# MoFHeka/MeepoEmbedding

Hardware: AMD Instinct MI355X
Metric: key-lookups/sec (higher is better)
Workload: dtype int64 keys / fp32 rows (copy)

## Files before the change

include/meepo_embedding.h:

```cpp
#ifndef MEEPO_EMBEDDING_H
#define MEEPO_EMBEDDING_H
#include <stddef.h>
#include <stdint.h>

#ifdef __cplusplus
extern "C" {
#endif

#define MEE_ABI_VERSION 2

#define MEE_EMPTY_KEY     INT64_MIN
#define MEE_RECLAIMED_KEY (INT64_MIN + 1)
#define MEE_BUCKET_WIDTH  16

enum { MEE_OK = 0, MEE_ERR_INVALID_ARG = -1, MEE_ERR_OUT_OF_MEMORY = -2, MEE_ERR_HIP = -3,
       MEE_ERR_NO_DEVICE = -4, MEE_ERR_BATCH_TOO_LARGE = -5, MEE_ERR_UNSUPPORTED = -6,
       MEE_ERR_RCCL = -7  };

enum { MEE_OPT_NONE = 0, MEE_OPT_ADAGRAD = 1, MEE_OPT_ADAM = 2 };
enum { MEE_INIT_CONSTANT = 0, MEE_INIT_UNIFORM = 1 };
enum { MEE_STATUS_TABLE_FULL = 1u, MEE_STATUS_RESERVED_KEY = 2u, MEE_STATUS_STALE_HANDLE = 4u, MEE_STATUS_INTERNAL = 8u };
enum { MEE_MEM_HBM = 0, MEE_MEM_HOST_PINNED = 1 };
enum { MEE_FLAG_TRACK_HITS = 1u, MEE_FLAG_ADMISSION = 2u };

// ... 153 lines not shown
int mee_apply_adam_indexed(mee_table* t, const int64_t* d_keys, const float* d_grads, size_t n_grad_rows, const uint32_t* d_grad_index,
                           size_t n, float lr, float beta1, float beta2, float eps, uint64_t step, void* stream);
int mee_apply_prepare(mee_table* t, const int64_t* d_keys, size_t n, void* stream);
int mee_apply_discard(mee_table* t, void* stream);
int mee_dedup_sum(mee_table* t, const int64_t* d_keys, const float* d_grads, size_t n, int64_t* d_uniq_out,
                  float* d_gsum_out, uint32_t* d_counts_out, int64_t* d_inverse_out, int64_t miss_index,
                  void* stream);

int mee_dedup_keys(mee_table* t, const int64_t* d_keys, size_t n, int64_t* d_uniq_out, int64_t* d_inverse_out, int64_t miss_index,
                   void* stream);

int mee_hash_batch(const int64_t* d_keys, size_t n, uint64_t n_buckets, uint32_t n_shards, uint64_t* d_mix_out,
                   uint64_t* d_bucket_out, uint32_t* d_owner_out, void* stream);
int mee_router_create(int32_t device, uint64_t max_batch, uint32_t n_shards, mee_router** out);
int mee_router_destroy(mee_router* r);
int mee_partition(mee_router* r, const int64_t* d_keys, size_t n, int64_t* d_send_keys, uint64_t* d_counts,
                  int64_t* d_perm, void* stream);
int mee_partition_padded(mee_router* r, const int64_t* d_keys, size_t n, int64_t* d_send_keys, uint64_t* d_counts,
                         int64_t* d_perm, void* stream);
int mee_scatter_rows(const void* d_rows, const int64_t* d_perm, size_t n, size_t row_bytes, void* d_out,
                     void* stream);
int mee_gather_rows(const void* d_rows, const int64_t* d_perm, size_t n, size_t row_bytes, void* d_out,
                    void* stream);

int mee_p2p_create(int32_t device, uint32_t n_shards, uint32_t rank, uint64_t slots_per_peer, uint64_t max_batch, uint32_t dim,
                   int with_payload, mee_p2p** out);
int mee_p2p_destroy(mee_p2p* c);
#define MEE_P2P_BUFFERS 6
int mee_p2p_export(mee_p2p* c, void* handles );
int mee_p2p_connect(mee_p2p* c, const void* all_handles );
int mee_p2p_buffers(mee_p2p* c, float** d_out, uint8_t** d_found);
int mee_p2p_push(mee_p2p* c, mee_router* r, const int64_t* d_send_keys, const int64_t* d_perm, const uint64_t* d_counts, size_t n,
                 void* stream);
int mee_p2p_find(mee_p2p* c, const mee_table* t, void* stream);
int mee_p2p_push_rows(mee_p2p* c, mee_router* r, const int64_t* d_send_keys, const int64_t* d_perm, const uint64_t* d_counts,
                      const float* d_rows, size_t n, void* stream);
int mee_p2p_inbox(mee_p2p* c, int64_t** d_keys, float** d_rows, uint64_t* n_slots);
int mee_p2p_barrier(mee_p2p* c, void* stream);
int mee_p2p_status(mee_p2p* c, uint32_t* bits_out, void* stream);


#define MEE_COMM_ID_BYTES 128
int mee_comm_unique_id(void* id_out );
int mee_comm_create(const void* id, uint32_t n_ranks, uint32_t rank, int32_t device, void** comm_out);
int mee_comm_destroy(void* comm);
int mee_comm_aborted(void* comm);
int mee_sharded_create(mee_table* local, void* nccl_comm, uint64_t max_batch ,
                       double pad_slack, mee_sharded** out);
enum { MEE_SHARDED_DEDUP = 1u };
typedef struct mee_sharded_options {
    uint32_t struct_size;
    uint32_t flags;
    uint64_t max_batch;
    double   pad_slack;
    mee_table* cold;
    uint64_t hot_key_limit;
} mee_sharded_options;
int mee_sharded_create_ex(mee_table* local, void* nccl_comm, const mee_sharded_options* options, mee_sharded** out);
int mee_sharded_destroy(mee_sharded* s);
int mee_sharded_info(const mee_sharded* s, uint32_t* n_shards, uint32_t* rank, uint64_t* segment_capacity );
int mee_sharded_find(mee_sharded* s, const int64_t* d_keys, size_t n, float* d_out, uint8_t* d_found , void* stream);
int mee_sharded_find_or_insert(mee_sharded* s, const int64_t* d_keys, size_t n, float* d_out, uint8_t* d_found, void* stream);
int mee_sharded_find_as(mee_sharded* s, const int64_t* d_keys, size_t n, void* d_out, uint32_t out_dtype, uint8_t* d_found , void* stream);
int mee_sharded_find_or_insert_as(mee_sharded* s, const int64_t* d_keys, size_t n, void* d_out, uint32_t out_dtype, uint8_t* d_found, void* stream);
int mee_sharded_traffic(const mee_sharded* s, uint64_t* sent_bytes, uint64_t* received_bytes);
int mee_sharded_insert(mee_sharded* s, const int64_t* d_keys, const float* d_values, size_t n, void* stream);
int mee_sharded_assign(mee_sharded* s, const int64_t* d_keys, const float* d_values, size_t n, uint8_t* d_found, void* stream);
int mee_sharded_remove(mee_sharded* s, const int64_t* d_keys, size_t n, uint8_t* d_found, void* stream);
int mee_sharded_apply_adagrad(mee_sharded* s, const int64_t* d_keys, const float* d_grads, size_t n, float lr, float eps, void* stream);
int mee_sharded_apply_adam(mee_sharded* s, const int64_t* d_keys, const float* d_grads, size_t n, float lr, float beta1, float beta2,
// ... 10 lines not shown
```

include/meepo_embedding.hpp:

```cpp
#pragma once
#include <cstdint>
#include <stdexcept>
#include <string>
#include <utility>

#include "meepo_embedding.h"

namespace meepo {

class Error : public std::runtime_error {
public:
    Error(int code, const std::string& msg) : std::runtime_error("meepo error " + std::to_string(code) + ": " + msg), code_(code) {}
    int code() const noexcept { return code_; }
private:
    int code_;
};

inline void check(int rc) {
    if (rc != MEE_OK) throw Error(rc, mee_last_error());
}

struct TableOptions {
    int32_t device = 0;
    uint64_t capacity = 0;
// ... 142 lines not shown
    }
    size_t size(void* stream = nullptr) const { return hot_.size(stream) + cold_.size(stream); }
private:
    Table hot_, cold_;
};

class Router {
public:
    Router(int32_t device, uint64_t max_batch, uint32_t n_shards) { check(mee_router_create(device, max_batch, n_shards, &r_)); }
    ~Router() { if (r_) mee_router_destroy(r_); }
    Router(Router&& o) noexcept : r_(std::exchange(o.r_, nullptr)) {}
    Router(const Router&) = delete;
    Router& operator=(const Router&) = delete;
    mee_router* handle() const noexcept { return r_; }
    void partition(const int64_t* d_keys, size_t n, int64_t* d_send_keys, uint64_t* d_counts, int64_t* d_perm, void* stream = nullptr) { check(mee_partition(r_, d_keys, n, d_send_keys, d_counts, d_perm, stream)); }
    void partition_padded(const int64_t* d_keys, size_t n, int64_t* d_send_keys, uint64_t* d_counts, int64_t* d_perm, void* stream = nullptr) { check(mee_partition_padded(r_, d_keys, n, d_send_keys, d_counts, d_perm, stream)); }
    static void scatter_rows(const void* d_rows, const int64_t* d_perm, size_t n, size_t row_bytes, void* d_out, void* stream = nullptr) { check(mee_scatter_rows(d_rows, d_perm, n, row_bytes, d_out, stream)); }
    static void gather_rows(const void* d_rows, const int64_t* d_perm, size_t n, size_t row_bytes, void* d_out, void* stream = nullptr) { check(mee_gather_rows(d_rows, d_perm, n, row_bytes, d_out, stream)); }
private:
    mee_router* r_ = nullptr;
};

class PeerExchange {
public:
    PeerExchange(int32_t device, uint32_t n_shards, uint32_t rank, uint64_t slots_per_peer, uint64_t max_batch, uint32_t dim, bool with_payload = false) {
        check(mee_p2p_create(device, n_shards, rank, slots_per_peer, max_batch, dim, with_payload ? 1 : 0, &c_));
    }
    ~PeerExchange() { if (c_) mee_p2p_destroy(c_); }
    PeerExchange(const PeerExchange&) = delete;
    PeerExchange& operator=(const PeerExchange&) = delete;
    void export_handles(void* handles_6x64) { check(mee_p2p_export(c_, handles_6x64)); }
    void connect(const void* all_handles_rank_major) { check(mee_p2p_connect(c_, all_handles_rank_major)); }
    void push(Router& r, const int64_t* d_send_keys, const int64_t* d_perm, const uint64_t* d_counts, size_t n, void* stream = nullptr) { check(mee_p2p_push(c_, r.handle(), d_send_keys, d_perm, d_counts, n, stream)); }
    void find(const Table& t, void* stream = nullptr) { check(mee_p2p_find(c_, t.handle(), stream)); }
    void barrier(void* stream = nullptr) { check(mee_p2p_barrier(c_, stream)); }
    void push_rows(Router& r, const int64_t* d_send_keys, const int64_t* d_perm, const uint64_t* d_counts, const float* d_rows, size_t n, void* stream = nullptr) {
        check(mee_p2p_push_rows(c_, r.handle(), d_send_keys, d_perm, d_counts, d_rows, n, stream));
    }
    int64_t* inbox_keys() const { int64_t* k = nullptr; check(mee_p2p_inbox(c_, &k, nullptr, nullptr)); return k; }
    float* inbox_rows() const { float* r = nullptr; check(mee_p2p_inbox(c_, nullptr, &r, nullptr)); return r; }
    uint64_t inbox_slots() const { uint64_t n = 0; check(mee_p2p_inbox(c_, nullptr, nullptr, &n)); return n; }
    float* rows() const { float* o = nullptr; check(mee_p2p_buffers(c_, &o, nullptr)); return o; }
    uint8_t* found() const { uint8_t* f = nullptr; check(mee_p2p_buffers(c_, nullptr, &f)); return f; }
    uint32_t status(void* stream = nullptr) { uint32_t b = 0; check(mee_p2p_status(c_, &b, stream)); return b; }
private:
    mee_p2p* c_ = nullptr;
};

class Communicator {
public:
    static void unique_id(void* id_128_bytes) { check(mee_comm_unique_id(id_128_bytes)); }
    Communicator(const void* id_128_bytes, uint32_t n_ranks, uint32_t rank, int32_t device) { check(mee_comm_create(id_128_bytes, n_ranks, rank, device, &c_)); }
    ~Communicator() { if (c_) mee_comm_destroy(c_); }
    Communicator(const Communicator&) = delete;
    Communicator& operator=(const Communicator&) = delete;
    void* handle() const noexcept { return c_; }
private:
    void* c_ = nullptr;
};

class ShardedTable {
public:
    ShardedTable(Table& local, void* nccl_comm, uint64_t max_batch, double pad_slack = 0.0) { check(mee_sharded_create(local.handle(), nccl_comm, max_batch, pad_slack, &s_)); }
    ShardedTable(Table& local, void* nccl_comm, uint64_t max_batch, double pad_slack, Table* cold, uint32_t flags = 0, uint64_t hot_key_limit = 0) {
        mee_sharded_options o{};
        o.struct_size = sizeof o; o.flags = flags; o.max_batch = max_batch; o.pad_slack = pad_slack; o.cold = cold ? cold->handle() : nullptr; o.hot_key_limit = hot_key_limit;
        check(mee_sharded_create_ex(local.handle(), nccl_comm, &o, &s_));
    }
    ~ShardedTable() { if (s_) mee_sharded_destroy(s_); }
    ShardedTable(const ShardedTable&) = delete;
    ShardedTable& operator=(const ShardedTable&) = delete;
    void find(const int64_t* d_keys, size_t n, float* d_out, uint8_t* d_found = nullptr, void* stream = nullptr) { check(mee_sharded_find(s_, d_keys, n, d_out, d_found, stream)); }
    void find_or_insert(const int64_t* d_keys, size_t n, float* d_out, uint8_t* d_found = nullptr, void* stream = nullptr) { check(mee_sharded_find_or_insert(s_, d_keys, n, d_out, d_found, stream)); }
// ... 17 lines not shown
```

meepoembedding_amd/_lib.py:

```python
from __future__ import annotations

import ctypes as C
import os

import torch

_HERE = os.path.dirname(os.path.abspath(__file__))
LIB_PATH = os.environ.get("MEE_LIB_PATH") or os.path.join(_HERE, "libmeepo_hip.so")

OK = 0
ERR_INVALID_ARG, ERR_OUT_OF_MEMORY, ERR_HIP, ERR_NO_DEVICE, ERR_BATCH_TOO_LARGE, ERR_UNSUPPORTED, ERR_RCCL = -1, -2, -3, -4, -5, -6, -7
OPT_NONE, OPT_ADAGRAD, OPT_ADAM = 0, 1, 2
INIT_CONSTANT, INIT_UNIFORM = 0, 1
STATUS_TABLE_FULL, STATUS_RESERVED_KEY, STATUS_STALE_HANDLE, STATUS_INTERNAL = 1, 2, 4, 8
FIND_DEFAULT, FIND_STREAM_STORES, FIND_CACHED_STORES, FIND_STREAM_ROWS, FIND_STREAM_BUCKETS = 0, 1, 2, 4, 8
HANDLE_SLOT_MASK = (1 << 40) - 1
MEM_HBM, MEM_HOST_PINNED = 0, 1
DTYPE_F32, DTYPE_BF16 = 0, 1
FLAG_TRACK_HITS, FLAG_ADMISSION = 1, 2
ABI_VERSION = 2
EMPTY_KEY = -(1 << 63)
RECLAIMED_KEY = EMPTY_KEY + 1
BUCKET_WIDTH = 16

# ... 99 lines not shown
    "mee_find_located": (C.c_int, [_vp, _vp, _sz, _vp, _vp, _vp, _vp]),
    "mee_find_or_insert_located": (C.c_int, [_vp, _vp, _sz, _vp, _vp, _vp, _vp]),
    "mee_find_located_prepare": (C.c_int, [_vp, _vp, _sz, _vp, _vp, _vp, _vp]),
    "mee_find_or_insert_located_prepare": (C.c_int, [_vp, _vp, _sz, _vp, _vp, _vp, _vp]),
    "mee_apply_adagrad_located": (C.c_int, [_vp, _vp, _vp, _vp, _sz, _f32, _f32, _vp]),
    "mee_apply_adam_located": (C.c_int, [_vp, _vp, _vp, _vp, _sz, _f32, _f32, _f32, _f32, _u64, _vp]),
    "mee_find_or_insert_admit": (C.c_int, [_vp, _vp, _sz, _vp, _vp, _u32, _vp]),
    "mee_admission_decay": (C.c_int, [_vp, _u32, _vp]),
    "mee_locate": (C.c_int, [_vp, _vp, _sz, _vp, _vp, _vp]),
    "mee_table_plane": (C.c_int, [_vp, _u32, C.POINTER(_vp), C.POINTER(_u64), C.POINTER(_u32)]),
    "mee_device_calibration": (C.c_int, [C.c_int32, C.POINTER(Calibration)]),
    "mee_probe_length": (C.c_int, [_vp, _vp, _sz, C.POINTER(_u64), _vp]),
    "mee_probe_histogram": (C.c_int, [_vp, _vp, _sz, C.POINTER(C.c_uint64), _vp]),
    "mee_apply_adagrad": (C.c_int, [_vp, _vp, _vp, _sz, _f32, _f32, _vp]),
    "mee_apply_adam": (C.c_int, [_vp, _vp, _vp, _sz, _f32, _f32, _f32, _f32, _u64, _vp]),
    "mee_apply_prepare": (C.c_int, [_vp, _vp, _sz, _vp]),
    "mee_apply_discard": (C.c_int, [_vp, _vp]),
    "mee_dedup_sum": (C.c_int, [_vp, _vp, _vp, _sz, _vp, _vp, _vp, _vp, C.c_int64, _vp]),
    "mee_hash_batch": (C.c_int, [_vp, _sz, _u64, _u32, _vp, _vp, _vp, _vp]),
    "mee_router_create": (C.c_int, [_i32, _u64, _u32, C.POINTER(_vp)]),
    "mee_router_destroy": (C.c_int, [_vp]),
    "mee_partition_padded": (C.c_int, [_vp, _vp, _sz, _vp, _vp, _vp, _vp]),
    "mee_partition": (C.c_int, [_vp, _vp, _sz, _vp, _vp, _vp, _vp]),
    "mee_p2p_create": (C.c_int, [_i32, _u32, _u32, _u64, _u64, _u32, C.c_int, C.POINTER(_vp)]),
    "mee_p2p_barrier": (C.c_int, [_vp, _vp]),
    "mee_p2p_push_rows": (C.c_int, [_vp, _vp, _vp, _vp, _vp, _vp, _sz, _vp]),
    "mee_p2p_inbox": (C.c_int, [_vp, C.POINTER(_vp), C.POINTER(_vp), C.POINTER(_u64)]),
    "mee_p2p_destroy": (C.c_int, [_vp]),
    "mee_p2p_export": (C.c_int, [_vp, _vp]),
    "mee_p2p_connect": (C.c_int, [_vp, _vp]),
    "mee_p2p_buffers": (C.c_int, [_vp, C.POINTER(_vp), C.POINTER(_vp)]),
    "mee_p2p_push": (C.c_int, [_vp, _vp, _vp, _vp, _vp, _sz, _vp]),
    "mee_p2p_find": (C.c_int, [_vp, _vp, _vp]),
    "mee_p2p_status": (C.c_int, [_vp, C.POINTER(_u32), _vp]),
    "mee_scatter_rows": (C.c_int, [_vp, _vp, _sz, _sz, _vp, _vp]),
    "mee_gather_rows": (C.c_int, [_vp, _vp, _sz, _sz, _vp, _vp]),
    "mee_comm_unique_id": (C.c_int, [_vp]),
    "mee_comm_create": (C.c_int, [_vp, _u32, _u32, _i32, C.POINTER(_vp)]),
    "mee_comm_destroy": (C.c_int, [_vp]),
    "mee_comm_aborted": (C.c_int, [_vp]),
    "mee_sharded_create": (C.c_int, [_vp, _vp, _u64, C.c_double, C.POINTER(_vp)]),
    "mee_sharded_create_ex": (C.c_int, [_vp, _vp, C.POINTER(ShardedOptions), C.POINTER(_vp)]),
    "mee_sharded_clear_status": (C.c_int, [_vp, _vp]),
    "mee_sharded_destroy": (C.c_int, [_vp]),
    "mee_sharded_info": (C.c_int, [_vp, C.POINTER(_u32), C.POINTER(_u32), C.POINTER(_u64)]),
    "mee_sharded_find": (C.c_int, [_vp, _vp, _sz, _vp, _vp, _vp]),
    "mee_sharded_find_or_insert": (C.c_int, [_vp, _vp, _sz, _vp, _vp, _vp]),
    "mee_sharded_find_as": (C.c_int, [_vp, _vp, _sz, _vp, _u32, _vp, _vp]),
    "mee_sharded_find_or_insert_as": (C.c_int, [_vp, _vp, _sz, _vp, _u32, _vp, _vp]),
    "mee_sharded_traffic": (C.c_int, [_vp, C.POINTER(_u64), C.POINTER(_u64)]),
    "mee_sharded_insert": (C.c_int, [_vp, _vp, _vp, _sz, _vp]),
    "mee_sharded_assign": (C.c_int, [_vp, _vp, _vp, _sz, _vp, _vp]),
    "mee_sharded_remove": (C.c_int, [_vp, _vp, _sz, _vp, _vp]),
    "mee_sharded_apply_adagrad": (C.c_int, [_vp, _vp, _vp, _sz, _f32, _f32, _vp]),
    "mee_sharded_apply_adam": (C.c_int, [_vp, _vp, _vp, _sz, _f32, _f32, _f32, _f32, _u64, _vp]),
    "mee_sharded_size": (C.c_int, [_vp, C.POINTER(_sz), _vp]),
    "mee_sharded_status": (C.c_int, [_vp, C.POINTER(_u32), _vp]),
}

_lib = None


def lib() -> C.CDLL:
    global _lib
    if _lib is None:
        if not os.path.exists(LIB_PATH):
# ... 29 lines not shown
```

meepoembedding_amd/csrc/meepo_router.hip:

```cpp
#include <hip/hip_runtime.h>

#include <cstdlib>
#include <cstring>
#include <new>

#include "meepo_device.h"
#include "meepo_host.h"

struct mee_router {
    int device;
    uint64_t max_batch;
    uint32_t n_shards;
    uint32_t max_blocks;
    uint32_t* blockcnt;
    uint64_t* base;
};

struct mee_p2p {
    int device;
    uint32_t n_shards, rank, dim;
    uint64_t cap, max_batch;
    int64_t* inbox_keys;
    int32_t* inbox_dst;
    uint32_t* inbox_cnt;
    float* out;
    uint8_t* found;
    float* inbox_rows;
    uint32_t* status;
    void** d_tables;
    void* h_tables[6][64];
    bool connected;
};

namespace mee {

constexpr int kPartBlock = 1024;
constexpr int kMaxShards = 64;

__global__ void hash_batch_kernel(const int64_t* __restrict__ keys, uint64_t n, uint64_t nb, uint32_t g, uint64_t* mix_out,
                                  uint64_t* bucket_out, uint32_t* owner_out) {
    for (uint64_t i = blockIdx.x * (uint64_t)blockDim.x + threadIdx.x; i < n; i += (uint64_t)gridDim.x * blockDim.x) {
        const int64_t k = keys[i];
        if (mix_out) mix_out[i] = mix64((uint64_t)k);
        if (bucket_out) bucket_out[i] = bucket_of(k, nb);
        if (owner_out) owner_out[i] = owner_of(k, g);
    }
}

template <bool SKIP_PAD>
__global__ __launch_bounds__(kPartBlock) void part_count_kernel(const int64_t* __restrict__ keys, uint32_t n, uint32_t g,
                                                                uint32_t* blockcnt) {
    __shared__ uint32_t wcnt[kPartBlock / 64][kMaxShards];
    const uint32_t i = blockIdx.x * kPartBlock + threadIdx.x;
    const int lane = threadIdx.x & 63, w = threadIdx.x >> 6;
    const int64_t key = i < n ? keys[i] : kEmpty;
    const bool inb = i < n && !(SKIP_PAD && key == kEmpty);
    const uint32_t o = inb ? owner_of(key, g) : 0xFFFFFFFFu;
    for (uint32_t p = 0; p < g; ++p) {
        const uint64_t m = __ballot(o == p);
        if (lane == 0) wcnt[w][p] = (uint32_t)__popcll(m);
    }
    __syncthreads();
    if (threadIdx.x < g) {
        uint32_t c = 0;
#pragma unroll
        for (int ww = 0; ww < kPartBlock / 64; ++ww) c += wcnt[ww][threadIdx.x];
        blockcnt[(uint64_t)blockIdx.x * g + threadIdx.x] = c;
    }
}

__global__ __launch_bounds__(1024) void part_scan_kernel(uint32_t* blockcnt, uint32_t n_blocks, uint32_t g, uint64_t* base,
                                                         uint64_t* counts_out) {
    __shared__ uint64_t total[kMaxShards];
    const int lane = threadIdx.x & 63, w = threadIdx.x >> 6, nw = blockDim.x >> 6;
    for (uint32_t p = w; p < g; p += nw) {
        uint32_t run = 0;
        for (uint32_t b0 = 0; b0 < n_blocks; b0 += 64) {
            const uint32_t b = b0 + lane;
            const uint32_t c = b < n_blocks ? blockcnt[(uint64_t)b * g + p] : 0;
            uint32_t incl = c;
#pragma unroll
            for (int d = 1; d < 64; d <<= 1) {
                const uint32_t t = __shfl_up(incl, d);
                if (lane >= d) incl += t;
            }
            if (b < n_blocks) blockcnt[(uint64_t)b * g + p] = run + incl - c;
            run += __shfl(incl, 63);
        }
        if (lane == 0) total[p] = run;
    }
    __syncthreads();
    if (threadIdx.x == 0) {
        uint64_t acc = 0;
        for (uint32_t p = 0; p < g; ++p) {
            base[p] = acc;
            counts_out[p] = total[p];
            acc += total[p];
        }
    }
}

template <bool SKIP_PAD>
__global__ __launch_bounds__(kPartBlock) void part_scatter_kernel(const int64_t* __restrict__ keys, uint32_t n, uint32_t g,
                                                                  const uint32_t* __restrict__ blockoff,
                                                                  const uint64_t* __restrict__ base, int64_t* send_keys,
                                                                  int64_t* perm) {
    __shared__ uint32_t wcnt[kPartBlock / 64][kMaxShards];
    const uint32_t i = blockIdx.x * kPartBlock + threadIdx.x;
    const int lane = threadIdx.x & 63, w = threadIdx.x >> 6;
    const int64_t key = i < n ? keys[i] : kEmpty;
    const bool inb = i < n && !(SKIP_PAD && key == kEmpty);
    const uint32_t o = inb ? owner_of(key, g) : 0xFFFFFFFFu;
    uint32_t r = 0;
    for (uint32_t p = 0; p < g; ++p) {
        const uint64_t m = __ballot(o == p);
        if (o == p) r = (uint32_t)__popcll(m & ((1ull << lane) - 1));
        if (lane == 0) wcnt[w][p] = (uint32_t)__popcll(m);
    }
    __syncthreads();
    if (inb) {
        for (int ww = 0; ww < w; ++ww) r += wcnt[ww][o];
        const uint64_t dst = base[o] + blockoff[(uint64_t)blockIdx.x * g + o] + r;
        send_keys[dst] = key;
        perm[dst] = (int64_t)i;
    }
}

template <typename T, bool SCATTER>
__global__ void permute_rows_kernel(const T* __restrict__ rows, const int64_t* __restrict__ perm, uint64_t n, uint32_t epr,
                                    T* __restrict__ out) {
    const uint64_t total = n * epr;
    for (uint64_t idx = blockIdx.x * (uint64_t)blockDim.x + threadIdx.x; idx < total; idx += (uint64_t)gridDim.x * blockDim.x) {
        const uint64_t q = idx / epr;
        const uint32_t e = (uint32_t)(idx - q * epr);
        const uint64_t p = (uint64_t)perm[q];
        if (SCATTER) out[p * epr + e] = rows[idx];
        else out[idx] = rows[p * epr + e];
    }
}

template <bool SCATTER>
static int permute_rows(const void* d_rows, const int64_t* d_perm, size_t n, size_t row_bytes, void* d_out, void* stream,
                        const char* name) {
    if (n && (!d_rows || !d_perm || !d_out)) return fail(MEE_ERR_INVALID_ARG, "%s: null argument", name);
    if (n == 0 || row_bytes == 0) return MEE_OK;
    hipStream_t st = (hipStream_t)stream;
    const bool a16 = row_bytes % 16 == 0 && ((uintptr_t)d_rows % 16 == 0) && ((uintptr_t)d_out % 16 == 0);
    const bool a4 = row_bytes % 4 == 0 && ((uintptr_t)d_rows % 4 == 0) && ((uintptr_t)d_out % 4 == 0);
    if (a16) {
        const uint32_t epr = (uint32_t)(row_bytes / 16);
        permute_rows_kernel<float4, SCATTER><<<grid_for(n * epr, 256, 1u << 16), 256, 0, st>>>((const float4*)d_rows, d_perm, n, epr, (float4*)d_out);
    } else if (a4) {
        const uint32_t epr = (uint32_t)(row_bytes / 4);
        permute_rows_kernel<uint32_t, SCATTER><<<grid_for(n * epr, 256, 1u << 16), 256, 0, st>>>((const uint32_t*)d_rows, d_perm, n, epr, (uint32_t*)d_out);
    } else {
        const uint32_t epr = (uint32_t)row_bytes;
        permute_rows_kernel<uint8_t, SCATTER><<<grid_for(n * epr, 256, 1u << 16), 256, 0, st>>>((const uint8_t*)d_rows, d_perm, n, epr, (uint8_t*)d_out);
    }
    MEE_HIP(hipGetLastError());
    return MEE_OK;
}

constexpr int kP2PBuffers = 6;
struct P2PPeers {
    int64_t** keys; int32_t** dst; uint32_t** cnt; float** out; uint8_t** found; float** rows;
};

__global__ __launch_bounds__(256) void p2p_push_kernel(const int64_t* __restrict__ send_keys, const int64_t* __restrict__ perm,
                                                       const uint64_t* __restrict__ counts, const uint64_t* __restrict__ base,
                                                       P2PPeers peers, uint32_t me, uint64_t cap, uint32_t* status, int pad) {
    const uint32_t p = blockIdx.y;
    const uint64_t cnt = counts[p];
    const uint64_t take = cnt < cap ? cnt : cap;
    int64_t* __restrict__ dk = peers.keys[p] + (uint64_t)me * cap;
    int32_t* __restrict__ dd = peers.dst[p] + (uint64_t)me * cap;
    const uint64_t b0 = base[p];
    for (uint64_t j = blockIdx.x * (uint64_t)blockDim.x + threadIdx.x; j < take; j += (uint64_t)gridDim.x * blockDim.x) {
        dk[j] = send_keys[b0 + j];
        dd[j] = (int32_t)perm[b0 + j];
    }
    if (pad)
        for (uint64_t j = take + blockIdx.x * (uint64_t)blockDim.x + threadIdx.x; j < cap; j += (uint64_t)gridDim.x * blockDim.x) dk[j] = kEmpty;
    if (blockIdx.x == 0 && threadIdx.x == 0) {
        peers.cnt[p][me] = (uint32_t)take;
        if (cnt > cap) atomicOr(status, 1u);
    }
}

__global__ __launch_bounds__(64) void p2p_barrier_kernel(P2PPeers peers, uint32_t me, uint32_t n_shards, uint32_t* status,
                                                         unsigned long long timeout_ticks) {
    const uint32_t q = threadIdx.x;
    uint32_t epoch = 0;
    if (q == 0) { epoch = status[1] + 1; status[1] = epoch; }
    epoch = __shfl(epoch, 0);
    if (q < n_shards) {
        uint32_t* theirs = peers.cnt[q] + n_shards + me;
        __hip_atomic_store(theirs, epoch, __ATOMIC_RELEASE, __HIP_MEMORY_SCOPE_SYSTEM);
        const uint32_t* mine = peers.cnt[me] + n_shards + q;
        const unsigned long long t0 = wall_clock64();
        while ((int32_t)(__hip_atomic_load(mine, __ATOMIC_ACQUIRE, __HIP_MEMORY_SCOPE_SYSTEM) - epoch) < 0) {
            if (wall_clock64() - t0 > timeout_ticks) { atomicOr(status, 2u); break; }
            __builtin_amdgcn_s_sleep(8);
        }
    }
}

__global__ __launch_bounds__(256) void p2p_push_rows_kernel(const float4* __restrict__ rows, const int64_t* __restrict__ perm,
                                                            const uint64_t* __restrict__ counts, const uint64_t* __restrict__ base,
                                                            P2PPeers peers, uint32_t me, uint64_t cap, uint32_t dim4) {
    const int lane = threadIdx.x & 63, tile = lane >> 4, tl = lane & 15;
    const uint32_t p = blockIdx.y;
    const uint64_t cnt = counts[p];
    const uint64_t take = cnt < cap ? cnt : cap;
    float4* __restrict__ dr = reinterpret_cast<float4*>(peers.rows[p]) + (uint64_t)me * cap * dim4;
    const uint64_t b0 = base[p];
    const uint64_t wave = (uint64_t)blockIdx.x * (blockDim.x >> 6) + (threadIdx.x >> 6), n_waves = (uint64_t)gridDim.x * (blockDim.x >> 6);
    for (uint64_t j0 = wave * 4; j0 < take; j0 += n_waves * 4) {
        const uint64_t j = j0 + tile;
// ... 136 lines not shown
static int partition_common(mee_router* r, const int64_t* d_keys, size_t n, int64_t* d_send_keys, uint64_t* d_counts, int64_t* d_perm,
                            void* stream, bool skip_pad, const char* name) {
    if (!r || !d_counts || (n && (!d_keys || !d_send_keys || !d_perm))) return fail(MEE_ERR_INVALID_ARG, "%s: null argument", name);
    if (n > r->max_batch) return fail(MEE_ERR_BATCH_TOO_LARGE, "%s: n=%zu exceeds max_batch=%llu", name, n, (unsigned long long)r->max_batch);
    DeviceGuard g(r->device);
    hipStream_t st = (hipStream_t)stream;
    const uint32_t nblk = (uint32_t)((n + kPartBlock - 1) / kPartBlock);
    if (nblk) with_flag(skip_pad, [&](auto sp) { part_count_kernel<sp><<<nblk, kPartBlock, 0, st>>>(d_keys, (uint32_t)n, r->n_shards, r->blockcnt); });
    part_scan_kernel<<<1, 1024, 0, st>>>(r->blockcnt, nblk, r->n_shards, r->base, d_counts);
    if (nblk) with_flag(skip_pad, [&](auto sp) { part_scatter_kernel<sp><<<nblk, kPartBlock, 0, st>>>(d_keys, (uint32_t)n, r->n_shards, r->blockcnt, r->base, d_send_keys, d_perm); });
    MEE_HIP(hipGetLastError());
    return MEE_OK;
}
int mee_partition(mee_router* r, const int64_t* d_keys, size_t n, int64_t* d_send_keys, uint64_t* d_counts, int64_t* d_perm,
                  void* stream) {
    MEE_RANGE("mee_partition");
    return partition_common(r, d_keys, n, d_send_keys, d_counts, d_perm, stream, false, "mee_partition");
}
int mee_partition_padded(mee_router* r, const int64_t* d_keys, size_t n, int64_t* d_send_keys, uint64_t* d_counts, int64_t* d_perm,
                         void* stream) {
    MEE_RANGE("mee_partition_padded");
    return partition_common(r, d_keys, n, d_send_keys, d_counts, d_perm, stream, true, "mee_partition_padded");
}

int mee_p2p_destroy(mee_p2p* c) {
    MEE_RANGE("mee_p2p_destroy");
    if (!c) return MEE_OK;
    DeviceGuard g(c->device);
    (void)hipDeviceSynchronize();
    if (c->connected)
        for (int b = 0; b < kP2PBuffers; ++b)
            for (uint32_t p = 0; p < c->n_shards; ++p)
                if (p != c->rank && c->h_tables[b][p]) (void)hipIpcCloseMemHandle(c->h_tables[b][p]);
    void* mine[] = {c->inbox_keys, c->inbox_dst, c->inbox_cnt, c->out, c->found, c->inbox_rows, c->status, c->d_tables};
    for (void* p : mine) if (p) (void)hipFree(p);
    delete c;
    return MEE_OK;
}

int mee_p2p_create(int32_t device, uint32_t n_shards, uint32_t rank, uint64_t slots_per_peer, uint64_t max_batch, uint32_t dim,
                   int with_payload, mee_p2p** out) {
    MEE_RANGE("mee_p2p_create");
    if (!out) return fail(MEE_ERR_INVALID_ARG, "mee_p2p_create: null out");
    *out = nullptr;
    if (n_shards == 0 || n_shards > (uint32_t)kMaxShards || rank >= n_shards || slots_per_peer == 0 || max_batch == 0 ||
        max_batch > (1ull << 30) || dim < 4 || (dim & 3))
        return fail(MEE_ERR_INVALID_ARG, "mee_p2p_create: bad arguments");
    int ndev = 0;
    if (hipGetDeviceCount(&ndev) != hipSuccess || ndev <= 0) return fail(MEE_ERR_NO_DEVICE, "mee_p2p_create: no HIP device visible");
    if (device < 0 || device >= ndev) return fail(MEE_ERR_INVALID_ARG, "mee_p2p_create: device %d out of range", device);
    DeviceGuard g(device);
    mee_p2p* c = new (std::nothrow) mee_p2p();
    if (!c) return fail(MEE_ERR_OUT_OF_MEMORY, "host allocation failed");
    memset(c, 0, sizeof *c);
    c->device = device; c->n_shards = n_shards; c->rank = rank; c->dim = dim; c->cap = slots_per_peer; c->max_batch = max_batch;
    const uint64_t slots = (uint64_t)n_shards * slots_per_peer;
    const bool fine = getenv("MEE_P2P_COARSE") == nullptr;
    auto sym_alloc = [&](void** p, size_t bytes) {
        return fine ? hipExtMallocWithFlags(p, bytes, hipDeviceMallocFinegrained) : hipMalloc(p, bytes);
    };
    if (sym_alloc((void**)&c->inbox_keys, slots * 8) != hipSuccess || sym_alloc((void**)&c->inbox_dst, slots * 4) != hipSuccess ||
        sym_alloc((void**)&c->inbox_cnt, 2 * n_shards * 4) != hipSuccess || sym_alloc((void**)&c->out, (max_batch + 1) * (uint64_t)dim * 4) != hipSuccess ||
        sym_alloc((void**)&c->found, max_batch + 1) != hipSuccess ||
        (with_payload && sym_alloc((void**)&c->inbox_rows, slots * (uint64_t)dim * 4) != hipSuccess) ||
        hipMalloc((void**)&c->status, 8) != hipSuccess ||
        hipMalloc((void**)&c->d_tables, kP2PBuffers * (size_t)n_shards * sizeof(void*)) != hipSuccess) {
        mee_p2p_destroy(c);
        return fail(MEE_ERR_OUT_OF_MEMORY, "mee_p2p_create: device allocation failed (%s)", fine ? "fine-grained" : "coarse-grained");
    }
    if (hipMemset(c->inbox_cnt, 0, 2 * n_shards * 4) != hipSuccess || hipMemset(c->status, 0, 8) != hipSuccess) {
        mee_p2p_destroy(c);
        return fail(MEE_ERR_HIP, "mee_p2p_create: hipMemset failed");
    }
    *out = c;
    return MEE_OK;
}

static void* p2p_local(const mee_p2p* c, int b) {
    switch (b) { case 0: return c->inbox_keys; case 1: return c->inbox_dst; case 2: return c->inbox_cnt; case 3: return c->out; case 4: return c->found; default: return c->inbox_rows; }
}

int mee_p2p_export(mee_p2p* c, void* handles) {
    MEE_RANGE("mee_p2p_export");
    if (!c || !handles) return fail(MEE_ERR_INVALID_ARG, "mee_p2p_export: null argument");
    static_assert(sizeof(hipIpcMemHandle_t) == MEE_IPC_HANDLE_BYTES, "IPC handle size");
    DeviceGuard g(c->device);
    memset(handles, 0, (size_t)kP2PBuffers * MEE_IPC_HANDLE_BYTES);
    for (int b = 0; b < kP2PBuffers; ++b) {
        if (!p2p_local(c, b)) continue;
        hipIpcMemHandle_t h;
        MEE_HIP(hipIpcGetMemHandle(&h, p2p_local(c, b)));
        memcpy((char*)handles + b * MEE_IPC_HANDLE_BYTES, &h, MEE_IPC_HANDLE_BYTES);
    }
    return MEE_OK;
}

int mee_p2p_connect(mee_p2p* c, const void* all_handles) {
    MEE_RANGE("mee_p2p_connect");
    if (!c || !all_handles) return fail(MEE_ERR_INVALID_ARG, "mee_p2p_connect: null argument");
    if (c->connected) return fail(MEE_ERR_INVALID_ARG, "mee_p2p_connect: already connected");
    DeviceGuard g(c->device);
    for (uint32_t p = 0; p < c->n_shards; ++p)
        for (int b = 0; b < kP2PBuffers; ++b) {
// ... 11 lines not shown
}

int mee_p2p_buffers(mee_p2p* c, float** d_out, uint8_t** d_found) {
    if (!c) return fail(MEE_ERR_INVALID_ARG, "mee_p2p_buffers: null argument");
    if (d_out) *d_out = c->out;
    if (d_found) *d_found = c->found;
    return MEE_OK;
}

static P2PPeers p2p_peers(const mee_p2p* c) {
    P2PPeers pp;
    pp.keys = (int64_t**)(c->d_tables + 0 * (size_t)c->n_shards);
    pp.dst = (int32_t**)(c->d_tables + 1 * (size_t)c->n_shards);
    pp.cnt = (uint32_t**)(c->d_tables + 2 * (size_t)c->n_shards);
    pp.out = (float**)(c->d_tables + 3 * (size_t)c->n_shards);
    pp.found = (uint8_t**)(c->d_tables + 4 * (size_t)c->n_shards);
    pp.rows = (float**)(c->d_tables + 5 * (size_t)c->n_shards);
    return pp;
}

int mee_p2p_push(mee_p2p* c, mee_router* r, const int64_t* d_send_keys, const int64_t* d_perm, const uint64_t* d_counts, size_t n,
                 void* stream) {
    MEE_RANGE("mee_p2p_push");
    if (!c || !r || !d_counts || (n && (!d_send_keys || !d_perm))) return fail(MEE_ERR_INVALID_ARG, "mee_p2p_push: null argument");
    if (!c->connected) return fail(MEE_ERR_INVALID_ARG, "mee_p2p_push: not connected");
    if (r->n_shards != c->n_shards || n > c->max_batch) return fail(MEE_ERR_INVALID_ARG, "mee_p2p_push: router/batch mismatch");
    DeviceGuard g(c->device);
    const dim3 grid(grid_for(n / c->n_shards + 256, 256, 1024), c->n_shards);
    p2p_push_kernel<<<grid, 256, 0, (hipStream_t)stream>>>(d_send_keys, d_perm, d_counts, r->base, p2p_peers(c), c->rank, c->cap, c->status, 0);
    MEE_HIP(hipGetLastError());
    return MEE_OK;
}

int mee_p2p_push_rows(mee_p2p* c, mee_router* r, const int64_t* d_send_keys, const int64_t* d_perm, const uint64_t* d_counts,
                      const float* d_rows, size_t n, void* stream) {
    MEE_RANGE("mee_p2p_push_rows");
    if (!c || !r || !d_counts || (n && (!d_send_keys || !d_perm))) return fail(MEE_ERR_INVALID_ARG, "mee_p2p_push_rows: null argument");
    if (!c->connected || !c->inbox_rows) return fail(MEE_ERR_INVALID_ARG, "mee_p2p_push_rows: context not connected or created without payload");
    if (r->n_shards != c->n_shards || n > c->max_batch) return fail(MEE_ERR_INVALID_ARG, "mee_p2p_push_rows: router/batch mismatch");
    DeviceGuard g(c->device);
    hipStream_t st = (hipStream_t)stream;
    const dim3 gk(grid_for(c->cap, 256, 1024), c->n_shards);
    p2p_push_kernel<<<gk, 256, 0, st>>>(d_send_keys, d_perm, d_counts, r->base, p2p_peers(c), c->rank, c->cap, c->status, 1);
    if (d_rows) {
        const dim3 gr(grid_for(n / c->n_shards + 64, 16, 4096), c->n_shards);
        p2p_push_rows_kernel<<<gr, 256, 0, st>>>((const float4*)d_rows, d_perm, d_counts, r->base, p2p_peers(c), c->rank, c->cap, c->dim / 4);
    }
    MEE_HIP(hipGetLastError());
    return MEE_OK;
}

int mee_p2p_inbox(mee_p2p* c, int64_t** d_keys, float** d_rows, uint64_t* n_slots) {
    if (!c) return fail(MEE_ERR_INVALID_ARG, "mee_p2p_inbox: null argument");
    if (d_keys) *d_keys = c->inbox_keys;
    if (d_rows) *d_rows = c->inbox_rows;
    if (n_slots) *n_slots = (uint64_t)c->n_shards * c->cap;
    return MEE_OK;
}

int mee_p2p_find(mee_p2p* c, const mee_table* t, void* stream) {
    MEE_RANGE("mee_p2p_find");
    if (!c || !t) return fail(MEE_ERR_INVALID_ARG, "mee_p2p_find: null argument");
    if (!c->connected) return fail(MEE_ERR_INVALID_ARG, "mee_p2p_find: not connected");
    const TableView v = table_view(t);
    if (v.dim != c->dim || v.device != c->device) return fail(MEE_ERR_INVALID_ARG, "mee_p2p_find: table dim/device mismatch");
    DeviceGuard g(c->device);
    const dim3 grid(grid_for(c->cap, 32, 1u << 16), c->n_shards);
    hipStream_t st = (hipStream_t)stream;
    with_row_shape(v.dim4, [&](auto d4) {
        p2p_find_kernel<d4, RowShape<d4>::rows_per_tile><<<grid, 256, 0, st>>>(v.keys, (const float4*)v.values, v.nb, v.dim4, v.default_value, c->inbox_keys,
                                                                               c->inbox_dst, c->inbox_cnt, p2p_peers(c), c->cap);
    });
    MEE_HIP(hipGetLastError());
    return MEE_OK;
}

int mee_p2p_barrier(mee_p2p* c, void* stream) {
    MEE_RANGE("mee_p2p_barrier");
    if (!c) return fail(MEE_ERR_INVALID_ARG, "mee_p2p_barrier: null argument");
    if (!c->connected) return fail(MEE_ERR_INVALID_ARG, "mee_p2p_barrier: not connected");
    DeviceGuard g(c->device);
    p2p_barrier_kernel<<<1, 64, 0, (hipStream_t)stream>>>(p2p_peers(c), c->rank, c->n_shards, c->status, 500000000ull);
    MEE_HIP(hipGetLastError());
    return MEE_OK;
}

int mee_p2p_status(mee_p2p* c, uint32_t* bits_out, void* stream) {
    MEE_RANGE("mee_p2p_status");
    if (!c || !bits_out) return fail(MEE_ERR_INVALID_ARG, "mee_p2p_status: null argument");
// ... 17 lines not shown
```

meepoembedding_amd/p2p.py:

```python
from __future__ import annotations

import ctypes as C

import torch
import torch.distributed as dist

from . import _lib
from ._lib import check


class _Raw:

    def __init__(self, ptr: int, shape, typestr: str):
        self.__cuda_array_interface__ = {"shape": tuple(shape), "typestr": typestr, "data": (ptr, False), "version": 2}


class PeerShardedFind:
    def __init__(self, local, router, max_batch: int, group=None, slack: float = 1.25, payload: bool = False,
                 device_barrier: bool = True):
        self.local, self.router, self.group = local, router, group
        self.world, self.rank = dist.get_world_size(group), dist.get_rank(group)
        self.device, self.dim, self.max_batch = local.device, local.dim, max_batch
        if router.n_shards != self.world:
            raise ValueError("router shards != process group size")
# ... 43 lines not shown
        if int(ok.item()) == 0:
            if self._h:
                _lib.lib().mee_p2p_destroy(self._h)
                self._h = None
            raise _lib.MeepoError(_lib.ERR_HIP, f"peer-to-peer set-up failed on some rank during {what}: {err!r}")

    def close(self) -> None:
        if getattr(self, "_h", None):
            try:
                self._barrier()
            except Exception:
                pass
            _lib.lib().mee_p2p_destroy(self._h)
            self._h = None

    def _barrier(self) -> None:
        if self.device_barrier and self._h:
            check(_lib.lib().mee_p2p_barrier(self._h, torch.cuda.current_stream(self.device).cuda_stream))
        elif self._staged:
            torch.cuda.synchronize(self.device)
            dist.barrier(group=self.group)
        else:
            dist.all_reduce(self._tok, group=self.group)

    def find(self, keys: torch.Tensor, check_overflow: bool = True, dedup: bool = False):
        keys = keys.contiguous().view(-1)
        n = keys.numel()
        if n > self.max_batch:
            raise _lib.MeepoError(_lib.ERR_BATCH_TOO_LARGE, f"n={n} exceeds max_batch={self.max_batch}")
        L = _lib.lib()
        s = torch.cuda.current_stream(self.device).cuda_stream
        if dedup:
            uniq, inverse = self.local.dedup_keys(keys, miss_index=self.max_batch)
            send_keys, counts, perm = self.router.partition(uniq, skip_padding=True)
            check(L.mee_p2p_push(self._h, self.router._h, send_keys.data_ptr(), perm.data_ptr(), counts.data_ptr(), n, s))
            self._barrier()
            check(L.mee_p2p_find(self._h, self.local._h, s))
            self._barrier()
            if check_overflow:
                self.check()
            rows = self.router.gather_rows(self.out, inverse, n_out=n)
            found = self.router.gather_rows(self.found, inverse, n_out=n)
            return rows, found
        send_keys, counts, perm = self.router.partition(keys)
        check(L.mee_p2p_push(self._h, self.router._h, send_keys.data_ptr(), perm.data_ptr(), counts.data_ptr(), n, s))
        self._barrier()
        check(L.mee_p2p_find(self._h, self.local._h, s))
        self._barrier()
        if check_overflow:
            self.check()
        return self.out[:n], self.found[:n]

    def find_or_insert(self, keys: torch.Tensor, check_overflow: bool = True):
        if not self.payload:
            raise _lib.MeepoError(_lib.ERR_INVALID_ARG, "find_or_insert needs PeerShardedFind(..., payload=True)")
        keys = keys.contiguous().view(-1)
        n = keys.numel()
        if n > self.max_batch:
            raise _lib.MeepoError(_lib.ERR_BATCH_TOO_LARGE, f"n={n} exceeds max_batch={self.max_batch}")
        L = _lib.lib()
        s = torch.cuda.current_stream(self.device).cuda_stream
        send_keys, counts, perm = self.router.partition(keys)
        check(L.mee_p2p_push_rows(self._h, self.router._h, send_keys.data_ptr(), perm.data_ptr(), counts.data_ptr(), None, n, s))
        self._barrier()
        self.local.find_or_insert(self.inbox_keys, out=self.inbox_rows, found=self._ensure_found)
        check(L.mee_p2p_find(self._h, self.local._h, s))
        self._barrier()
        if check_overflow:
            self.check()
        return self.out[:n], self.found[:n]

    def _deliver(self, keys: torch.Tensor, rows: torch.Tensor, aggregate: bool = False) -> None:
        if not self.payload:
            raise _lib.MeepoError(_lib.ERR_INVALID_ARG, "mutators need PeerShardedFind(..., payload=True)")
        keys = keys.contiguous().view(-1)
        n = keys.numel()
        rows = rows.contiguous().view(n, -1)
        if n > self.max_batch or rows.shape[1] != self.dim or rows.dtype != torch.float32:
# ... 48 lines not shown
```

Baseline: 7.825 billion.

## Fuse partition and peer push into single-pass decoupled-lookback kernel

Adds a single kernel that ranks keys by owner shard, computes each chunk's per-shard offset with a decoupled look-back prefix scan, and writes keys plus destination indices straight into the peers' inboxes. The Python find path now calls it in place of the separate router partition (count, scan, scatter) plus push. This removes several kernel launches and the intermediate send_keys/perm buffers with their round trip through HBM. In exchange it relies on chunks being claimed in order via an atomic ticket and on spin-waits over a device look-back array, with epoch-tagged words, a wrap-reset path and a timeout that sets a status bit.

```diff
diff --git a/include/meepo_embedding.h b/include/meepo_embedding.h
--- a/include/meepo_embedding.h
+++ b/include/meepo_embedding.h
@@ -209,10 +209,12 @@
 int mee_p2p_buffers(mee_p2p* c, float** d_out, uint8_t** d_found);
 int mee_p2p_push(mee_p2p* c, mee_router* r, const int64_t* d_send_keys, const int64_t* d_perm, const uint64_t* d_counts, size_t n,
                  void* stream);
+int mee_p2p_partition_push(mee_p2p* c, const int64_t* d_keys, size_t n, int skip_pad, void* stream);
 int mee_p2p_find(mee_p2p* c, const mee_table* t, void* stream);
 int mee_p2p_push_rows(mee_p2p* c, mee_router* r, const int64_t* d_send_keys, const int64_t* d_perm, const uint64_t* d_counts,
                       const float* d_rows, size_t n, void* stream);
 int mee_p2p_inbox(mee_p2p* c, int64_t** d_keys, float** d_rows, uint64_t* n_slots);
+int mee_p2p_inbox_index(mee_p2p* c, int32_t** d_dst, uint32_t** d_counts);
 int mee_p2p_barrier(mee_p2p* c, void* stream);
 int mee_p2p_status(mee_p2p* c, uint32_t* bits_out, void* stream);
 
diff --git a/include/meepo_embedding.hpp b/include/meepo_embedding.hpp
--- a/include/meepo_embedding.hpp
+++ b/include/meepo_embedding.hpp
@@ -198,6 +198,7 @@
     void export_handles(void* handles_6x64) { check(mee_p2p_export(c_, handles_6x64)); }
     void connect(const void* all_handles_rank_major) { check(mee_p2p_connect(c_, all_handles_rank_major)); }
     void push(Router& r, const int64_t* d_send_keys, const int64_t* d_perm, const uint64_t* d_counts, size_t n, void* stream = nullptr) { check(mee_p2p_push(c_, r.handle(), d_send_keys, d_perm, d_counts, n, stream)); }
+    void partition_push(const int64_t* d_keys, size_t n, bool skip_pad = false, void* stream = nullptr) { check(mee_p2p_partition_push(c_, d_keys, n, skip_pad ? 1 : 0, stream)); }
     void find(const Table& t, void* stream = nullptr) { check(mee_p2p_find(c_, t.handle(), stream)); }
     void barrier(void* stream = nullptr) { check(mee_p2p_barrier(c_, stream)); }
     void push_rows(Router& r, const int64_t* d_send_keys, const int64_t* d_perm, const uint64_t* d_counts, const float* d_rows, size_t n, void* stream = nullptr) {
@@ -205,6 +206,8 @@
     }
     int64_t* inbox_keys() const { int64_t* k = nullptr; check(mee_p2p_inbox(c_, &k, nullptr, nullptr)); return k; }
     float* inbox_rows() const { float* r = nullptr; check(mee_p2p_inbox(c_, nullptr, &r, nullptr)); return r; }
+    int32_t* inbox_dst() const { int32_t* d = nullptr; check(mee_p2p_inbox_index(c_, &d, nullptr)); return d; }
+    uint32_t* inbox_counts() const { uint32_t* n = nullptr; check(mee_p2p_inbox_index(c_, nullptr, &n)); return n; }
     uint64_t inbox_slots() const { uint64_t n = 0; check(mee_p2p_inbox(c_, nullptr, nullptr, &n)); return n; }
     float* rows() const { float* o = nullptr; check(mee_p2p_buffers(c_, &o, nullptr)); return o; }
     uint8_t* found() const { uint8_t* f = nullptr; check(mee_p2p_buffers(c_, nullptr, &f)); return f; }
diff --git a/meepoembedding_amd/_lib.py b/meepoembedding_amd/_lib.py
--- a/meepoembedding_amd/_lib.py
+++ b/meepoembedding_amd/_lib.py
@@ -155,6 +155,8 @@
     "mee_p2p_buffers": (C.c_int, [_vp, C.POINTER(_vp), C.POINTER(_vp)]),
     "mee_p2p_push": (C.c_int, [_vp, _vp, _vp, _vp, _vp, _sz, _vp]),
     "mee_p2p_find": (C.c_int, [_vp, _vp, _vp]),
+    "mee_p2p_partition_push": (C.c_int, [_vp, _vp, _sz, C.c_int, _vp]),
+    "mee_p2p_inbox_index": (C.c_int, [_vp, C.POINTER(_vp), C.POINTER(_vp)]),
     "mee_p2p_status": (C.c_int, [_vp, C.POINTER(_u32), _vp]),
     "mee_scatter_rows": (C.c_int, [_vp, _vp, _sz, _sz, _vp, _vp]),
     "mee_gather_rows": (C.c_int, [_vp, _vp, _sz, _sz, _vp, _vp]),
diff --git a/meepoembedding_amd/csrc/meepo_router.hip b/meepoembedding_amd/csrc/meepo_router.hip
--- a/meepoembedding_amd/csrc/meepo_router.hip
+++ b/meepoembedding_amd/csrc/meepo_router.hip
@@ -27,6 +27,8 @@
     uint8_t* found;
     float* inbox_rows;
     uint32_t* status;
+    unsigned long long* fuse;
+    uint32_t max_chunks;
     void** d_tables;
     void* h_tables[6][64];
     bool connected;
@@ -48,18 +50,29 @@
 }
 
 template <bool SKIP_PAD>
+__device__ __forceinline__ uint32_t part_wave_ranks(const int64_t* __restrict__ keys, uint32_t n, uint32_t g, uint32_t blk,
+                                                    uint32_t (*wcnt)[kMaxShards], int64_t& key, uint32_t& o) {
+    const uint32_t i = blk * kPartBlock + threadIdx.x;
+    const int lane = threadIdx.x & 63, w = threadIdx.x >> 6;
+    key = i < n ? keys[i] : kEmpty;
+    const bool inb = i < n && !(SKIP_PAD && key == kEmpty);
+    o = inb ? owner_of(key, g) : 0xFFFFFFFFu;
+    uint32_t r = 0;
+    for (uint32_t p = 0; p < g; ++p) {
+        const uint64_t m = __ballot(o == p);
+        if (o == p) r = (uint32_t)__popcll(m & ((1ull << lane) - 1));
+        if (lane == 0) wcnt[w][p] = (uint32_t)__popcll(m);
+    }
+    return r;
+}
+
+template <bool SKIP_PAD>
 __global__ __launch_bounds__(kPartBlock) void part_count_kernel(const int64_t* __restrict__ keys, uint32_t n, uint32_t g,
                                                                 uint32_t* blockcnt) {
     __shared__ uint32_t wcnt[kPartBlock / 64][kMaxShards];
-    const uint32_t i = blockIdx.x * kPartBlock + threadIdx.x;
-    const int lane = threadIdx.x & 63, w = threadIdx.x >> 6;
-    const int64_t key = i < n ? keys[i] : kEmpty;
-    const bool inb = i < n && !(SKIP_PAD && key == kEmpty);
-    const uint32_t o = inb ? owner_of(key, g) : 0xFFFFFFFFu;
-    for (uint32_t p = 0; p < g; ++p) {
-        const uint64_t m = __ballot(o == p);
-        if (lane == 0) wcnt[w][p] = (uint32_t)__popcll(m);
-    }
+    int64_t key;
+    uint32_t o;
+    part_wave_ranks<SKIP_PAD>(keys, n, g, blockIdx.x, wcnt, key, o);
     __syncthreads();
     if (threadIdx.x < g) {
         uint32_t c = 0;
@@ -107,18 +120,12 @@
                                                                   int64_t* perm) {
     __shared__ uint32_t wcnt[kPartBlock / 64][kMaxShards];
     const uint32_t i = blockIdx.x * kPartBlock + threadIdx.x;
-    const int lane = threadIdx.x & 63, w = threadIdx.x >> 6;
-    const int64_t key = i < n ? keys[i] : kEmpty;
-    const bool inb = i < n && !(SKIP_PAD && key == kEmpty);
-    const uint32_t o = inb ? owner_of(key, g) : 0xFFFFFFFFu;
-    uint32_t r = 0;
-    for (uint32_t p = 0; p < g; ++p) {
-        const uint64_t m = __ballot(o == p);
-        if (o == p) r = (uint32_t)__popcll(m & ((1ull << lane) - 1));
-        if (lane == 0) wcnt[w][p] = (uint32_t)__popcll(m);
-    }
+    const int w = threadIdx.x >> 6;
+    int64_t key;
+    uint32_t o;
+    uint32_t r = part_wave_ranks<SKIP_PAD>(keys, n, g, blockIdx.x, wcnt, key, o);
     __syncthreads();
-    if (inb) {
+    if (o != 0xFFFFFFFFu) {
         for (int ww = 0; ww < w; ++ww) r += wcnt[ww][o];
         const uint64_t dst = base[o] + blockoff[(uint64_t)blockIdx.x * g + o] + r;
         send_keys[dst] = key;
@@ -184,6 +191,118 @@
     if (blockIdx.x == 0 && threadIdx.x == 0) {
         peers.cnt[p][me] = (uint32_t)take;
         if (cnt > cap) atomicOr(status, 1u);
+    }
+}
+
+__device__ __forceinline__ unsigned long long look_word(uint32_t epoch, bool prefix, uint32_t count) {
+    return ((unsigned long long)epoch << 32) | (prefix ? 0x80000000ull : 0ull) | count;
+}
+
+__device__ __forceinline__ unsigned long long look_wait(const unsigned long long* src, uint32_t epoch, uint32_t* status,
+                                                        unsigned long long timeout_ticks) {
+    unsigned long long wd = __hip_atomic_load(src, __ATOMIC_RELAXED, __HIP_MEMORY_SCOPE_AGENT);
+    if ((uint32_t)(wd >> 32) == epoch) return wd;
+    const unsigned long long t0 = wall_clock64();
+    while (true) {
+        __builtin_amdgcn_s_sleep(1);
+        wd = __hip_atomic_load(src, __ATOMIC_RELAXED, __HIP_MEMORY_SCOPE_AGENT);
+        if ((uint32_t)(wd >> 32) == epoch) return wd;
+        if (wall_clock64() - t0 > timeout_ticks) { atomicOr(status, 2u); return look_word(epoch, true, 0); }
+    }
+}
+
+constexpr int kPushTiles = 4;
+constexpr int kPushChunk = kPushTiles * kPartBlock;
+
+template <bool SKIP_PAD>
+__global__ __launch_bounds__(kPartBlock) void p2p_partition_push_kernel(const int64_t* __restrict__ keys, uint32_t n, uint32_t g, uint32_t n_chunks,
+                                                                        uint32_t max_chunks, P2PPeers peers, uint32_t me, uint64_t cap,
+                                                                        uint32_t* status, unsigned long long* ctl, uint32_t* epoch_p,
+                                                                        unsigned long long* look, unsigned long long timeout_ticks) {
+    __shared__ uint32_t wcnt[kPushTiles][kPartBlock / 64][kMaxShards];
+    __shared__ uint32_t tbase[kPushTiles][kMaxShards];
+    __shared__ uint32_t tot[kMaxShards], excl[kMaxShards];
+    __shared__ int64_t* seg_keys[kMaxShards];
+    __shared__ int32_t* seg_dst[kMaxShards];
+    __shared__ uint32_t s_chunk, s_epoch, s_wrap;
+    const int lane = threadIdx.x & 63, w = threadIdx.x >> 6;
+    if (threadIdx.x == 0) {
+        s_chunk = (uint32_t)__hip_atomic_fetch_add(ctl, 1ull, __ATOMIC_RELAXED, __HIP_MEMORY_SCOPE_AGENT);
+        s_epoch = __hip_atomic_load(epoch_p, __ATOMIC_RELAXED, __HIP_MEMORY_SCOPE_AGENT);
+        s_wrap = 0;
+    }
+    __syncthreads();
+    const uint32_t chunk = __builtin_amdgcn_readfirstlane(s_chunk), epoch = __builtin_amdgcn_readfirstlane(s_epoch);
+    if (chunk >= n_chunks) {
+        if (threadIdx.x == 0) atomicOr(status, 2u);
+        return;
+    }
+    int64_t key[kPushTiles];
+    uint32_t o[kPushTiles], r[kPushTiles];
+#pragma unroll
+    for (int t = 0; t < kPushTiles; ++t) r[t] = part_wave_ranks<SKIP_PAD>(keys, n, g, chunk * kPushTiles + t, wcnt[t], key[t], o[t]);
+    __syncthreads();
+    if (threadIdx.x < g) {
+        uint32_t c = 0;
+#pragma unroll
+        for (int t = 0; t < kPushTiles; ++t) {
+            tbase[t][threadIdx.x] = c;
+#pragma unroll
+            for (int ww = 0; ww < kPartBlock / 64; ++ww) c += wcnt[t][ww][threadIdx.x];
+        }
+        tot[threadIdx.x] = c;
+        __hip_atomic_store(look + (uint64_t)chunk * g + threadIdx.x, look_word(epoch, chunk == 0, c), __ATOMIC_RELAXED, __HIP_MEMORY_SCOPE_AGENT);
+        seg_keys[threadIdx.x] = peers.keys[threadIdx.x] + (uint64_t)me * cap;
+        seg_dst[threadIdx.x] = peers.dst[threadIdx.x] + (uint64_t)me * cap;
+    }
+    __syncthreads();
+    for (uint32_t p = w; p < g; p += kPartBlock / 64) {
+        uint32_t run = 0;
+        for (int64_t j0 = (int64_t)chunk - 1;; j0 -= 64) {
+            const int64_t j = j0 - lane;
+            const unsigned long long wd = j >= 0 ? look_wait(look + (uint64_t)j * g + p, epoch, status, timeout_ticks)
+                                                 : look_word(epoch, true, 0);
+            const uint64_t pre = __ballot((wd >> 31) & 1);
+            const int first = pre ? __ffsll((unsigned long long)pre) - 1 : 63;
+            uint32_t v = lane <= first ? (uint32_t)wd & 0x7FFFFFFFu : 0;
+#pragma unroll
+            for (int d = 32; d; d >>= 1) v += __shfl_xor(v, d);
+            run += v;
+            if (pre) break;
+        }
+        if (lane == 0) {
+            excl[p] = run;
+            if (chunk) __hip_atomic_store(look + (uint64_t)chunk * g + p, look_word(epoch, true, run + tot[p]), __ATOMIC_RELAXED, __HIP_MEMORY_SCOPE_AGENT);
+        }
+    }
+    __syncthreads();
+#pragma unroll
+    for (int t = 0; t < kPushTiles; ++t)
+        if (o[t] != 0xFFFFFFFFu) {
+            uint32_t off = excl[o[t]] + tbase[t][o[t]] + r[t];
+            for (int ww = 0; ww < w; ++ww) off += wcnt[t][ww][o[t]];
+            if (off < cap) {
+                seg_keys[o[t]][off] = key[t];
+                seg_dst[o[t]][off] = (int32_t)((chunk * kPushTiles + t) * kPartBlock + threadIdx.x);
+            }
+        }
+    if (chunk == n_chunks - 1 && threadIdx.x < g) {
+        const uint64_t cnt = (uint64_t)excl[threadIdx.x] + tot[threadIdx.x];
+        peers.cnt[threadIdx.x][me] = (uint32_t)(cnt < cap ? cnt : cap);
+        if (cnt > cap) atomicOr(status, 1u);
+    }
+    if (threadIdx.x == 0) {
+        const unsigned long long was = __hip_atomic_fetch_add(ctl, 1ull << 32, __ATOMIC_RELAXED, __HIP_MEMORY_SCOPE_AGENT);
+        if ((uint32_t)(was >> 32) == n_chunks - 1) {
+            __hip_atomic_store(ctl, 0ull, __ATOMIC_RELAXED, __HIP_MEMORY_SCOPE_AGENT);
+            if (epoch + 1 != 0) __hip_atomic_store(epoch_p, epoch + 1, __ATOMIC_RELAXED, __HIP_MEMORY_SCOPE_AGENT);
+            else s_wrap = 1;
+        }
+    }
+    __syncthreads();
+    if (s_wrap) {
+        for (uint64_t q = threadIdx.x; q < (uint64_t)max_chunks * g; q += kPartBlock) look[q] = 0;
+        if (threadIdx.x == 0) __hip_atomic_store(epoch_p, 1u, __ATOMIC_RELAXED, __HIP_MEMORY_SCOPE_AGENT);
     }
 }
 
@@ -386,7 +505,7 @@
         for (int b = 0; b < kP2PBuffers; ++b)
             for (uint32_t p = 0; p < c->n_shards; ++p)
                 if (p != c->rank && c->h_tables[b][p]) (void)hipIpcCloseMemHandle(c->h_tables[b][p]);
-    void* mine[] = {c->inbox_keys, c->inbox_dst, c->inbox_cnt, c->out, c->found, c->inbox_rows, c->status, c->d_tables};
+    void* mine[] = {c->inbox_keys, c->inbox_dst, c->inbox_cnt, c->out, c->found, c->inbox_rows, c->status, c->d_tables, c->fuse};
     for (void* p : mine) if (p) (void)hipFree(p);
     delete c;
     return MEE_OK;
@@ -409,6 +528,8 @@
     memset(c, 0, sizeof *c);
     c->device = device; c->n_shards = n_shards; c->rank = rank; c->dim = dim; c->cap = slots_per_peer; c->max_batch = max_batch;
     const uint64_t slots = (uint64_t)n_shards * slots_per_peer;
+    c->max_chunks = (uint32_t)((max_batch + kPushChunk - 1) / kPushChunk);
+    const size_t fuse_bytes = (2 + (size_t)c->max_chunks * n_shards) * 8;
     const bool fine = getenv("MEE_P2P_COARSE") == nullptr;
     auto sym_alloc = [&](void** p, size_t bytes) {
         return fine ? hipExtMallocWithFlags(p, bytes, hipDeviceMallocFinegrained) : hipMalloc(p, bytes);
@@ -417,12 +538,14 @@
         sym_alloc((void**)&c->inbox_cnt, 2 * n_shards * 4) != hipSuccess || sym_alloc((void**)&c->out, (max_batch + 1) * (uint64_t)dim * 4) != hipSuccess ||
         sym_alloc((void**)&c->found, max_batch + 1) != hipSuccess ||
         (with_payload && sym_alloc((void**)&c->inbox_rows, slots * (uint64_t)dim * 4) != hipSuccess) ||
-        hipMalloc((void**)&c->status, 8) != hipSuccess ||
+        hipMalloc((void**)&c->status, 8) != hipSuccess || hipMalloc((void**)&c->fuse, fuse_bytes) != hipSuccess ||
         hipMalloc((void**)&c->d_tables, kP2PBuffers * (size_t)n_shards * sizeof(void*)) != hipSuccess) {
         mee_p2p_destroy(c);
         return fail(MEE_ERR_OUT_OF_MEMORY, "mee_p2p_create: device allocation failed (%s)", fine ? "fine-grained" : "coarse-grained");
     }
-    if (hipMemset(c->inbox_cnt, 0, 2 * n_shards * 4) != hipSuccess || hipMemset(c->status, 0, 8) != hipSuccess) {
+    const unsigned long long first_epoch = 1;
+    if (hipMemset(c->inbox_cnt, 0, 2 * n_shards * 4) != hipSuccess || hipMemset(c->status, 0, 8) != hipSuccess ||
+        hipMemset(c->fuse, 0, fuse_bytes) != hipSuccess || hipMemcpy(c->fuse + 1, &first_epoch, 8, hipMemcpyHostToDevice) != hipSuccess) {
         mee_p2p_destroy(c);
         return fail(MEE_ERR_HIP, "mee_p2p_create: hipMemset failed");
     }
@@ -500,6 +623,21 @@
     return MEE_OK;
 }
 
+int mee_p2p_partition_push(mee_p2p* c, const int64_t* d_keys, size_t n, int skip_pad, void* stream) {
+    MEE_RANGE("mee_p2p_partition_push");
+    if (!c || (n && !d_keys)) return fail(MEE_ERR_INVALID_ARG, "mee_p2p_partition_push: null argument");
+    if (!c->connected) return fail(MEE_ERR_INVALID_ARG, "mee_p2p_partition_push: not connected");
+    if (n > c->max_batch) return fail(MEE_ERR_BATCH_TOO_LARGE, "mee_p2p_partition_push: n=%zu exceeds max_batch=%llu", n, (unsigned long long)c->max_batch);
+    DeviceGuard g(c->device);
+    const uint32_t n_chunks = n ? (uint32_t)((n + kPushChunk - 1) / kPushChunk) : 1;
+    with_flag(skip_pad != 0, [&](auto sp) {
+        p2p_partition_push_kernel<sp><<<n_chunks, kPartBlock, 0, (hipStream_t)stream>>>(d_keys, (uint32_t)n, c->n_shards, n_chunks, c->max_chunks, p2p_peers(c), c->rank, c->cap,
+                                                                                      c->status, c->fuse, (uint32_t*)(c->fuse + 1), c->fuse + 2, 500000000ull);
+    });
+    MEE_HIP(hipGetLastError());
+    return MEE_OK;
+}
+
 int mee_p2p_push_rows(mee_p2p* c, mee_router* r, const int64_t* d_send_keys, const int64_t* d_perm, const uint64_t* d_counts,
                       const float* d_rows, size_t n, void* stream) {
     MEE_RANGE("mee_p2p_push_rows");
@@ -523,6 +661,13 @@
     if (d_keys) *d_keys = c->inbox_keys;
     if (d_rows) *d_rows = c->inbox_rows;
     if (n_slots) *n_slots = (uint64_t)c->n_shards * c->cap;
+    return MEE_OK;
+}
+
+int mee_p2p_inbox_index(mee_p2p* c, int32_t** d_dst, uint32_t** d_counts) {
+    if (!c) return fail(MEE_ERR_INVALID_ARG, "mee_p2p_inbox_index: null argument");
+    if (d_dst) *d_dst = c->inbox_dst;
+    if (d_counts) *d_counts = c->inbox_cnt;
     return MEE_OK;
 }
 
diff --git a/meepoembedding_amd/p2p.py b/meepoembedding_amd/p2p.py
--- a/meepoembedding_amd/p2p.py
+++ b/meepoembedding_amd/p2p.py
@@ -99,8 +99,7 @@
         s = torch.cuda.current_stream(self.device).cuda_stream
         if dedup:
             uniq, inverse = self.local.dedup_keys(keys, miss_index=self.max_batch)
-            send_keys, counts, perm = self.router.partition(uniq, skip_padding=True)
-            check(L.mee_p2p_push(self._h, self.router._h, send_keys.data_ptr(), perm.data_ptr(), counts.data_ptr(), n, s))
+            check(L.mee_p2p_partition_push(self._h, uniq.data_ptr(), n, 1, s))
             self._barrier()
             check(L.mee_p2p_find(self._h, self.local._h, s))
             self._barrier()
@@ -109,8 +108,7 @@
             rows = self.router.gather_rows(self.out, inverse, n_out=n)
             found = self.router.gather_rows(self.found, inverse, n_out=n)
             return rows, found
-        send_keys, counts, perm = self.router.partition(keys)
-        check(L.mee_p2p_push(self._h, self.router._h, send_keys.data_ptr(), perm.data_ptr(), counts.data_ptr(), n, s))
+        check(L.mee_p2p_partition_push(self._h, keys.data_ptr(), n, 0, s))
         self._barrier()
         check(L.mee_p2p_find(self._h, self.local._h, s))
         self._barrier()
```

Result: no change. 7.810 billion, median of 2 (-0.2%).
